# salesforce/ai-economist

Hardware: AMD Instinct MI355X
Metric: agent-steps/sec, gather-trade-build 25x25 4-agent batched envs (higher is better)
Workload: dtype u8/i32 state + f64 coin/utility (f32 observations); 1 GPU; C2 BASELINE configs[1]: gather-trade-build 25x25, 4 agents + planner, Build+CDA+Gather+PeriodicBracketTax, 4096 replicas/GPU, uniform random policy, planner not counted; envs_per_gpu=4096, global_envs=4096, n_agents=4, kernel_specialisation=compile time, parallelism=single GPU

## Files before the change

ai-economist_amd/csrc/aie_capi.hip:

```cpp
#include <hip/hip_runtime.h>

#include <cstdio>
#include <cstdlib>
#include <cstring>
#include <vector>

#include "aie_kernels.hip"
#include "aie_kernels_sampler.hip"
#include "aie_kernels_rollout.hip"
#include "aie_kernels_ose.hip"
#include "aie_kernels_saez.hip"
#include "aie_kernels_ppo.hip"
#include "aie_kernels_mlp.hip"
#include "aie_kernels_mlp_bwd.hip"
#include "aie_kernels_covid.hip"
#include "aie_jit.h"
#include "aie_trainer_plan.h"

struct aie_env {
  aie_params P{};
  aie_params* d_params;
  aie_tensor_table tt;
  uint8_t* arena;
  bool owns_arena;
// ... 206 lines not shown
  } else {
    k = AIE_KERNEL(aie_step_kernel);
  }
  if (!k.name) return AIE_E_INVALID;
  *out = {k, !k.fn, (unsigned)(covid ? AIE_NT : ose ? OSE_NT : 2 * AIE_NT), env->lds};
  return AIE_OK;
}

static int aie_launch_step(aie_env* env, const aie_route<aie_step_fn>& r, unsigned grid, const int32_t* d_actions_a,
                           const int32_t* d_actions_p, const NextActions& next, hipStream_t st) {
  if (r.module) {
    const aie_params* dp = env->d_params;
    uint8_t* ar = env->arena;
    NextActions nx = next;
    void* args[] = {&dp, &ar, &d_actions_a, &d_actions_p, &nx};
    AIE_HIP_CHECK(env, hipModuleLaunchKernel(env->jit_step, grid, 1, 1, r.block, 1, 1, (unsigned)r.lds, st, args, nullptr));
  } else {
    hipLaunchKernelGGL(r.k.fn, dim3(grid), dim3(r.block), r.lds, st, env->d_params, env->arena, d_actions_a, d_actions_p, next);
  }
  return AIE_OK;
}

static unsigned aie_log_grid(const aie_env* env) {
  if (env->P.c.scenario != AIE_SCN_GTB || env->P.ev_replicas <= 0 || !env->log_active) return 0;
  const int64_t L = env->P.ev_replicas, E8 = env->P.E >> 3;
  return (env->P.E & 7) ? (unsigned)L : (L <= E8 ? (unsigned)(8 * (L - 1) + 1) : (unsigned)env->P.E);
}

static aie_route<aie_reset_fn> aie_select_reset(const aie_env* env) {
  const aie_params& P = env->P;
  if (P.c.scenario == AIE_SCN_COVID) return {AIE_KERNEL(aie_covid_reset_kernel), false, AIE_NT, 0};
  if (P.c.scenario == AIE_SCN_ONE_STEP_ECONOMY) return {{nullptr, "aie_ose_reset_kernel"}, false, OSE_NT, env->lds};
  const bool layout = P.c.layout_gen != AIE_LAYOUT_FIXED;
  aie_route<aie_reset_fn> r = {AIE_KERNEL(aie_reset_kernel), false, AIE_NT, env->lds + aie::layout_gen_lds_bytes(P)};
  if (layout) r.k = AIE_KERNEL(aie_reset_kernel_layout), r.block = LG_NW * AIE_NT;
  if (P.dev_skip_mask == 0 && !env->dev_generic) {
    if (env->spec == AIE_KERNEL_INSTANCE_JIT) r.k = {nullptr, "aie_jit_reset"}, r.module = true;
    else if (env->spec >= 0 && env->spec < AIE_N_SPECS && aie_spec_kernel.reset[env->spec].fn) r.k = aie_spec_kernel.reset[env->spec];
  }
  return r;
}

static void aie_launch_reset(aie_env* env, const uint8_t* d_mask, int keep_rewards, void* stream) {
  const aie_route<aie_reset_fn> r = aie_select_reset(env);
  const dim3 g((unsigned)env->P.E), b(r.block);
  hipStream_t st = static_cast<hipStream_t>(stream);
  if (r.module) {
    const aie_params* dp = env->d_params;
    uint8_t* ar = env->arena;
    void* args[] = {&dp, &ar, &d_mask, &keep_rewards};
    (void)hipModuleLaunchKernel(env->jit_reset, g.x, 1, 1, b.x, 1, 1, (unsigned)r.lds, st, args, nullptr);
  } else if (!r.k.fn) {
    hipLaunchKernelGGL(aie_ose_reset_kernel, g, b, r.lds, st, env->d_params, env->arena, d_mask);
  } else {
    hipLaunchKernelGGL(r.k.fn, g, b, r.lds, st, env->d_params, env->arena, d_mask, keep_rewards);
  }
  if (env->P.c.scenario == AIE_SCN_GTB && aie__layout_staged(&env->P.c)) {
    const int threshold = env->P.E >= 4 ? (int)(env->P.E / 4) : 1;
    hipLaunchKernelGGL(aie_layout_decide_kernel, dim3(1), dim3(1), 0, st, env->d_params, env->arena, threshold);
    hipLaunchKernelGGL(aie_layout_refill_kernel, g, dim3(LG_NW * AIE_NT), r.lds, st, env->d_params, env->arena);
  }
}

template <bool LOGP>
using aie_policy_fn = void (*)(const aie_sampler_args, uint8_t*, const float*, const float*, uint64_t, int64_t, int32_t*, int32_t*,
                               int, const SamplerLogp<LOGP>);
template <bool LOGP>
static aie_policy_fn<LOGP> aie_policy_sampler(const aie_sampler_args& S) {
// ... 872 lines not shown
```

ai-economist_amd/csrc/aie_device.h:

```cpp
#pragma once
#include <hip/hip_runtime.h>
#include <stdint.h>

#include "aie_layout.h"
#include "aie_glibc_math.h"

#pragma clang fp contract(off)

#ifdef AIE_JIT
#include "aie_jit_image.h"
#else
#include "aie_spec_generated.h"
#endif
template <int SPEC>
__device__ __forceinline__ const aie_params& aie_spec_params(const aie_params* run_time) {
  if constexpr (SPEC < 0) return *run_time;
  else return *reinterpret_cast<const aie_params*>(aie_spec_image<SPEC>::bytes);
}

#define AIE_NT 64
#define AIE_DIRTY_CAP 64

namespace aie {

// ... 612 lines not shown
  return v;
}
__device__ __forceinline__ int rng_permutation(MTL& l, int lane, int n) {
  int p = lane;
  for (int i = n - 1; i >= 1; --i) {
    const int j = (int)rng_interval(l, lane, (uint32_t)i);
    const int vi = bcast(p, i), vj = bcast(p, j);
    p = (lane == i) ? vj : ((lane == j) ? vi : p);
  }
  return p;
}
__device__ __forceinline__ double rng_gauss(const Ctx& c, MT& m) {
  int32_t* has = R_I32(c, o_mt_has_gauss);
  double* g = R_F64(c, o_mt_gauss);
  if (*has) {
    const double t = *g;
    *has = 0;
    *g = 0.0;
    return t;
  }
  double f, x1, x2, r2;
  do {
    x1 = 2.0 * rng_double(m, c.tid) - 1.0;
    x2 = 2.0 * rng_double(m, c.tid) - 1.0;
    r2 = x1 * x1 + x2 * x2;
  } while (r2 >= 1.0 || r2 == 0.0);
  f = sqrt(-2.0 * aie_log_glibc(r2) / r2);
  *g = f * x1;
  *has = 1;
  return f * x2;
}
__device__ __forceinline__ double rng_pareto(MT& m, int lane, double a) { return aie_exp_glibc(-aie_log_glibc(1.0 - rng_double(m, lane)) / a) - 1.0; }
__device__ __forceinline__ double rng_lognormal(const Ctx& c, MT& m, double mean, double sigma) { return aie_exp_glibc(mean + sigma * rng_gauss(c, m)); }

#pragma clang fp contract(off)
__device__ __forceinline__ double tax_curr_rate_max(const Ctx& c) {
  return aie_annealed_tax_limit(*R_I32(c, o_tax_last_completions), c.R.c.tax_annealing_warmup,
                                c.R.c.tax_annealing_slope, c.R.c.tax_rate_max);
}
__device__ __forceinline__ uint8_t* saez_block(const Ctx& c) {
  return C_MET(c) - c.R.a_metrics - (int64_t)c.e * c.P.met_bytes + c.R.a_saez + (int64_t)c.e * c.P.saez_stride;
}
__device__ __forceinline__ double tax_rate(const Ctx& c, int b) {
  if (c.P.c.tax_model == AIE_TAX_MODEL_WRAPPER) return c.rtab[R_I32(c, o_tax_rate_idx)[b]];
  if (c.saez) {
    const double r = R_F64(c, o_tax_saez_rates)[b];
    const double cap = c.P.c.tax_annealing ? tax_curr_rate_max(c) : c.R.c.tax_rate_max;
    return r < cap ? r : cap;
  }
  const double r = c.R.c.tax_fixed_rates[b];
  if (!c.P.c.tax_annealing) return r;
  const double cap = tax_curr_rate_max(c);
  return r < cap ? r : cap;
}
__device__ __forceinline__ double tax_rate_obs(const Ctx& c, int b) {
  if (c.saez) return R_F64(c, o_tax_saez_obs_rates)[b];
  return tax_rate(c, b);
}
__device__ __forceinline__ bool tax_rate_action_visible(const Ctx& c, int j) {
  if (!c.P.c.tax_annealing) return true;
  double full = 0;
  for (int k = 0; k < c.P.c.tax_n_disc_rates; ++k) full = fmax(full, fabs(c.rtab[k]));
  const double vis = aie_annealed_tax_limit(*R_I32(c, o_tax_last_completions), c.R.c.tax_annealing_warmup,
                                            c.R.c.tax_annealing_slope, full);
  return fabs(c.rtab[j]) <= vis;
}
// ... 67 lines not shown
```

ai-economist_amd/csrc/aie_kernels.hip:

```cpp
#pragma once
#include "aie_device.h"

namespace aie {
__device__ __forceinline__ bool can_agent_occupy(const Ctx& c, int r, int col, int agent) {
  if (r < 0 || r >= c.P.H || col < 0 || col >= c.P.W) return false;
  const int cell = r * c.P.W + col;
  const uint32_t w = R_CELLS(c)[cell];
  if (AIE_CELL_FLAGS(w) & AIE_CELL_WATER) return false;
  const int o = AIE_CELL_OWNER(w);
  if (!(o < 0 || o == agent)) return false;
  const int occ = c.locmap[cell];
  return occ == 0 || occ == agent + 1;
}

__device__ __forceinline__ void log_event(const Ctx& c, int type, int a1, int a2, int a3, int a4, int a5,
                                          int a6, int a7, int a8, double f) {
  if (c.tid != 0) return;
  const int k = c.srcn[2];
  if (k >= c.R.ev_cap) return;
  int32_t* row = c.ev + 4 + k * AIE_EV_WORDS;
  row[0] = type; row[1] = a1; row[2] = a2; row[3] = a3; row[4] = a4;
  row[5] = a5; row[6] = a6; row[7] = a7; row[8] = a8; row[9] = 0;
  *reinterpret_cast<double*>(row + 10) = f;
  c.srcn[2] = k + 1;
// ... 1106 lines not shown
  const uint32_t amap_bytes = (uint32_t)(n * c.P.am_ch * plane * 4), aidx_bytes = (uint32_t)(n * 2 * plane * 2);
  SpatialOut o;
  o.amap = make_rsrc(arena + c.R.a_obs_a_map + (int64_t)c.e * amap_bytes, amap_bytes);
  o.aidx = make_rsrc(arena + c.R.a_obs_a_idx + (int64_t)c.e * aidx_bytes, aidx_bytes);
  const bool pl = c.P.c.planner_gets_spatial_info != 0;
  o.pmap = make_rsrc(arena + c.R.a_obs_p_map + (int64_t)c.e * CM * HW * 4, pl ? (uint32_t)(CM * HW * 4) : 0u);
  o.pidx = make_rsrc(arena + c.R.a_obs_p_idx + (int64_t)c.e * 2 * HW * 2, pl ? (uint32_t)(2 * HW * 2) : 0u);
  return o;
}

template <bool WATER>
__device__ __forceinline__ void crop_item(const Ctx& c, const SpatialOut& o, int i, int d, int r, int col) {
  constexpr int CM = WATER ? 6 : 5;
  const int H = c.P.H, W = c.P.W, WV2 = c.P.WV * c.P.WV;
  const int so = i * (CM + 1) * WV2 * 4, si = i * 2 * WV2 * 2;
  const bool in = (r >= 0) & (r < H) & (col >= 0) & (col < W);
  const int cell = in ? r * W + col : 0;
  const uint32_t cw = in ? R_CELLS(c)[cell] : 0x00ff0000u;
  float ch[6];
  cell_channels<WATER>(cw, ch);
#pragma unroll
  for (int k = 0; k < CM; ++k) buf_store_f32(o.amap, ch[k], 4 * d, so + k * WV2 * 4);
  buf_store_f32(o.amap, in ? 1.0f : 0.0f, 4 * d, so + CM * WV2 * 4);
  const int own = AIE_CELL_OWNER(cw);
  int v0 = own >= 0 ? own + 2 : 0;
  int v1 = in ? (int)c.locmap[cell] : 0;
  v1 = v1 ? v1 + 1 : 0;
  if (v0 == i + 2) v0 = 1;
  if (v1 == i + 2) v1 = 1;
  buf_store_i16(o.aidx, v0, 2 * d, si);
  buf_store_i16(o.aidx, v1, 2 * d, si + WV2 * 2);
}
template <bool WATER>
__device__ __forceinline__ void crop_agent(const Ctx& c, const SpatialOut& o, int i) {
  const int WV = c.P.WV, WV2 = WV * WV, w = c.P.c.obs_range;
  const int r0 = R_I32(c, o_loc_r)[i] - w, c0 = R_I32(c, o_loc_c)[i] - w;
  for (int d = c.tid; d < WV2; d += AIE_NT) {
    const int dr = udiv(d, WV, c.P.mg_WV), dc = d - dr * WV;
    crop_item<WATER>(c, o, i, d, r0 + dr, c0 + dc);
  }
}
template <bool WATER>
__device__ __forceinline__ void planner_cell(const Ctx& c, const SpatialOut& o, int cell) {
  constexpr int CM = WATER ? 6 : 5;
  const int HW = c.P.HW;
  float ch[6];
  const uint32_t cw = R_CELLS(c)[cell];
  cell_channels<WATER>(cw, ch);
#pragma unroll
  for (int k = 0; k < CM; ++k) buf_store_f32(o.pmap, ch[k], 4 * cell, k * HW * 4);
  const int own = AIE_CELL_OWNER(cw);
  const int occ = c.locmap[cell];
  buf_store_i16(o.pidx, own >= 0 ? own + 2 : 0, 2 * cell, 0);
  buf_store_i16(o.pidx, occ ? occ + 1 : 0, 2 * cell, HW * 2);
}

template <bool WATER>
__device__ __forceinline__ void write_spatial_observations_t(const Ctx& c, uint8_t* __restrict__ arena) {
  constexpr int CM = WATER ? 6 : 5;
  const int n = c.P.n, HW = c.P.HW;
  const uint32_t* cells = R_CELLS(c);
  const SpatialOut o = spatial_out<WATER>(c, arena);
  if (c.P.c.full_observability) {
    const uint32_t* lm4f = reinterpret_cast<const uint32_t*>(c.locmap);
    for (int i = 0; i < n; ++i) {
      const int so = i * CM * HW * 4, si = i * 2 * HW * 2;
      for (int q = c.tid; q < (HW >> 2); q += AIE_NT) {
        const uint4 cw = reinterpret_cast<const uint4*>(cells)[q];
        const uint32_t cws[4] = {cw.x, cw.y, cw.z, cw.w};
        float ch[4][6];
#pragma unroll
        for (int u = 0; u < 4; ++u) cell_channels<WATER>(cws[u], ch[u]);
#pragma unroll
        for (int k = 0; k < CM; ++k) buf_store_f32x4(o.amap, ch[0][k], ch[1][k], ch[2][k], ch[3][k], 16 * q, so + k * HW * 4);
        const uint32_t occ4 = lm4f[q];
#pragma unroll
        for (int u = 0; u < 4; ++u) {
          const int own = AIE_CELL_OWNER(cws[u]);
          int v0 = own >= 0 ? own + 2 : 0;
          const int occ = (int)((occ4 >> (8 * u)) & 0xffu);
          int v1 = occ ? occ + 1 : 0;
          if (v0 == i + 2) v0 = 1;
          if (v1 == i + 2) v1 = 1;
          buf_store_i16(o.aidx, v0, 8 * q + 2 * u, si);
          buf_store_i16(o.aidx, v1, 8 * q + 2 * u, si + HW * 2);
        }
      }
      for (int cell = 4 * (HW >> 2) + c.tid; cell < HW; cell += AIE_NT) {
        float ch[6];
        const uint32_t cw = cells[cell];
        cell_channels<WATER>(cw, ch);
#pragma unroll
        for (int k = 0; k < CM; ++k) buf_store_f32(o.amap, ch[k], 4 * cell, so + k * HW * 4);
        const int own = AIE_CELL_OWNER(cw);
        int v0 = own >= 0 ? own + 2 : 0;
        const int occ = c.locmap[cell];
        int v1 = occ ? occ + 1 : 0;
        if (v0 == i + 2) v0 = 1;
        if (v1 == i + 2) v1 = 1;
        buf_store_i16(o.aidx, v0, 2 * cell, si);
        buf_store_i16(o.aidx, v1, 2 * cell, si + HW * 2);
      }
    }
  } else {
    for (int i = 0; i < n; ++i) crop_agent<WATER>(c, o, i);
  }
  if (c.P.c.planner_gets_spatial_info) {
    const int nq4 = HW >> 2;
    const uint32_t* lm4 = reinterpret_cast<const uint32_t*>(c.locmap);
    for (int q = c.tid; q < nq4; q += AIE_NT) {
      const uint4 cw = reinterpret_cast<const uint4*>(cells)[q];
      const uint32_t cws[4] = {cw.x, cw.y, cw.z, cw.w};
      float ch[4][6];
#pragma unroll
      for (int u = 0; u < 4; ++u) cell_channels<WATER>(cws[u], ch[u]);
#pragma unroll
      for (int k = 0; k < CM; ++k) buf_store_f32x4(o.pmap, ch[0][k], ch[1][k], ch[2][k], ch[3][k], 16 * q, k * HW * 4);
      const uint32_t occ4 = lm4[q];
      uint32_t ow[2], oc[2];
#pragma unroll
      for (int u = 0; u < 4; ++u) {
        const int own = AIE_CELL_OWNER(cws[u]);
        const uint32_t vo = (uint32_t)(own >= 0 ? own + 2 : 0);
        const uint32_t occ = (occ4 >> (8 * u)) & 0xffu;
        const uint32_t vc = occ ? occ + 1 : 0;
        if (u & 1) { ow[u >> 1] |= vo << 16; oc[u >> 1] |= vc << 16; }
        else { ow[u >> 1] = vo; oc[u >> 1] = vc; }
      }
      buf_store_u32x2(o.pidx, ow[0], ow[1], 8 * q, 0);
      if ((HW & 1) == 0) {
        buf_store_u32x2(o.pidx, oc[0], oc[1], 8 * q, HW * 2);
      } else {
#pragma unroll
        for (int u = 0; u < 4; ++u) buf_store_i16(o.pidx, (int)((oc[u >> 1] >> (16 * (u & 1))) & 0xffffu), 8 * q + 2 * u, HW * 2);
      }
    }
    for (int cell = 4 * nq4 + c.tid; cell < HW; cell += AIE_NT) planner_cell<WATER>(c, o, cell);
  }
}

template <bool WATER>
__device__ __forceinline__ void agent_full_cell(const Ctx& c, const SpatialOut& o, int i, int cell) {
  constexpr int CM = WATER ? 6 : 5;
  const int HW = c.P.HW;
  const int so = i * CM * HW * 4, si = i * 2 * HW * 2;
  float ch[6];
  const uint32_t cw = R_CELLS(c)[cell];
  cell_channels<WATER>(cw, ch);
#pragma unroll
  for (int k = 0; k < CM; ++k) buf_store_f32(o.amap, ch[k], 4 * cell, so + k * HW * 4);
  const int own = AIE_CELL_OWNER(cw);
  int v0 = own >= 0 ? own + 2 : 0;
  const int occ = c.locmap[cell];
  int v1 = occ ? occ + 1 : 0;
  if (v0 == i + 2) v0 = 1;
  if (v1 == i + 2) v1 = 1;
  buf_store_i16(o.aidx, v0, 2 * cell, si);
  buf_store_i16(o.aidx, v1, 2 * cell, si + HW * 2);
}

template <bool WATER>
__device__ __forceinline__ void update_spatial_observations_t(const Ctx& c, uint8_t* __restrict__ arena) {
  const int n = c.P.n, W = c.P.W, WV = c.P.WV, w = c.P.c.obs_range;
  const int cnt = uni(c.dirty[0]);
  if (cnt > AIE_DIRTY_CAP) {
    write_spatial_observations_t<WATER>(c, arena);
    return;
  }
  const SpatialOut o = spatial_out<WATER>(c, arena);
  const uint32_t mv0 = (uint32_t)uni(c.dirty[1]), mv1 = (uint32_t)uni(c.dirty[2]);
  const uint16_t* dl = dirty_list(c);
  const int cell = c.tid < cnt ? (int)dl[c.tid] : -1;
  const int r = cell >= 0 ? udiv(cell, W, c.P.mg_W) : 0, col = cell - r * W;
  for (int i = 0; i < n; ++i) {
    if (c.P.c.full_observability) {
      if (cell >= 0) agent_full_cell<WATER>(c, o, i, cell);
      continue;
    }
    const bool moved = ((i < 32 ? mv0 >> i : mv1 >> (i - 32)) & 1u) != 0;
    if (moved) {
      crop_agent<WATER>(c, o, i);
    } else if (cell >= 0) {
      const int dr = r - (R_I32(c, o_loc_r)[i] - w), dc = col - (R_I32(c, o_loc_c)[i] - w);
      if (dr >= 0 && dr < WV && dc >= 0 && dc < WV) crop_item<WATER>(c, o, i, dr * WV + dc, r, col);
    }
  }
  if (c.P.c.planner_gets_spatial_info && cell >= 0) planner_cell<WATER>(c, o, cell);
}
__device__ __forceinline__ void write_spatial_observations(const Ctx& c, uint8_t* __restrict__ arena) {
  if (c.P.c.has_water) write_spatial_observations_t<true>(c, arena);
  else write_spatial_observations_t<false>(c, arena);
}
__device__ __forceinline__ void update_spatial_observations(const Ctx& c, uint8_t* __restrict__ arena) {
  if (c.P.c.has_water) update_spatial_observations_t<true>(c, arena);
  else update_spatial_observations_t<false>(c, arena);
}

__device__ __forceinline__ void flat_a(const BufRsrc& aflat, int idx, float v) { buf_store_f32(aflat, v, 4 * idx, 0); }

__device__ __forceinline__ float flat_time_value(const Ctx& c) {
  const int t = *R_I32(c, o_timestep);
  return (float)((double)t / (c.P.c.allow_observation_scaling ? (double)c.R.c.episode_length : 1.0));
}

struct AgentScalars {
  double coin; int inv0, inv1, lr, lc;
  __device__ __forceinline__ AgentScalars(const Ctx& c, int i)
      : coin(R_F64(c, o_inv_coin)[i]), inv0(R_I32(c, o_inv_res)[i]), inv1(R_I32(c, o_inv_res)[c.P.n + i]),
        lr(R_I32(c, o_loc_r)[i]), lc(R_I32(c, o_loc_c)[i]) {}
  __device__ __forceinline__ void write(const Ctx& c, uint8_t* __restrict__ arena, const BufRsrc& aflat, float* q, int i,
                                        float tval, double isc) const {
    const aie_params& P = c.P;
    const int f0 = i * P.FA;
    flat_a(aflat, f0 + P.fa_time, tval);
    const float w0 = (float)(coin * isc);
    const float w1 = (float)((double)inv0 * isc);
    const float w2 = (float)((double)inv1 * isc);
    const float w3 = (float)((double)lc / (double)P.W);
    const float w4 = (float)((double)lr / (double)P.H);
    flat_a(aflat, f0 + P.fa_world + 0, w0); flat_a(aflat, f0 + P.fa_world + 1, w1); flat_a(aflat, f0 + P.fa_world + 2, w2);
    if (!P.c.full_observability) {
      flat_a(aflat, f0 + P.fa_world + 3, w3); flat_a(aflat, f0 + P.fa_world + 4, w4);
      q[P.fpa_world + 0] = w0; q[P.fpa_world + 1] = w1; q[P.fpa_world + 2] = w2;
      if (P.c.planner_gets_spatial_info) { q[P.fpa_world + 3] = w3; q[P.fpa_world + 4] = w4; }
// ... 1054 lines not shown
        LG_ACC(4);
      }
    }
    happy = true;
    for (int q = 0; q < 2; ++q) {
      const int rs = q == 0 ? 1 : 0;
      int count = 0;
      for (int base = 0; base < HW; base += NT) {
        const int cell = base + gtid;
        count += lg_block_count(cell < HW && mbp[rs][cell], sh, par, wave, lane);
      }
      const double ratio = ((double)count / (double)HW) / c.R.c.layout_coverage[rs];
      if (!((1 / 1.4) <= ratio && ratio <= 1.4)) happy = false;
    }
  }
  mt_copy(m, s3.w[0]);
  m.pos = s3.pos;
  if (stage_out) {
    for (int cell = gtid; cell < HW; cell += NT) stage_out[cell] = (uint8_t)((mbp[0][cell] ? 1u : 0u) | (mbp[1][cell] ? 2u : 0u));
  } else {
    layout_install(c, gtid, NT, [&](int cell) -> uint32_t { return (mbp[0][cell] ? 1u : 0u) | (mbp[1][cell] ? 2u : 0u); });
  }
  __syncthreads();
#ifdef AIE_DEV
  if (c.R.dev_trace && gtid == 0) {
    lg_acc[0] = wall_clock64() - lg_start;
    for (int k = 0; k < 8; ++k) c.R.dev_trace[12 * c.e + k] = lg_acc[k];
  }
#endif
}
}

namespace aie {
template <int SPEC, bool LAYOUT = true>
__device__ __forceinline__ void reset_body(const aie_params* __restrict__ params, uint8_t* __restrict__ arena,
                                           const uint8_t* __restrict__ mask, int keep_rewards, uint8_t* lds) {
  const aie_params& R = *params;
  const aie_params& P = aie_spec_params<SPEC>(params);
  const int e = replica_of_block((int)blockIdx.x, R.E);
  if (mask && !mask[e]) return;
  const int gtid = (int)threadIdx.x, wave = gtid >> 6, nwaves = (int)blockDim.x >> 6;
  const Ctx c = make_ctx(P, R, lds, e, gtid & 63, arena);
  const int n = P.n, HW = P.HW, tid = c.tid;
  if (wave == 0) {
    for (int q = tid; q < (P.met_bytes >> 2); q += AIE_NT) reinterpret_cast<uint32_t*>(C_MET(c))[q] = 0u;
    if (c.ev && tid == 0) c.ev[0] = 0;
  }
  MT m;
  mt_init(m, P);
  load_record(c, arena, m, wave, nwaves, wave);
  __syncthreads();
  m.pos = uni(*R_I32(c, o_mt_pos));
  mt_fast_attach(c, m);
  if (LAYOUT && P.c.layout_gen != AIE_LAYOUT_FIXED) {
    if (aie__layout_staged(&P.c)) {
      uint32_t st[4];
#pragma unroll
      for (int k = 0; k < 4; ++k) st[k] = (uint32_t)uni((int)R_U32(c, o_mt)[k]);
      const uint64_t tag = aie_layout_tag(st);
      const uint64_t* tags = reinterpret_cast<const uint64_t*>(arena + R.a_layout_tag);
      int32_t* ctl = reinterpret_cast<int32_t*>(arena + R.a_layout_ctl);
      const uint64_t have = tags[e];
      const bool staged = (uint32_t)uni((int)(uint32_t)have) == (uint32_t)tag && (uint32_t)uni((int)(uint32_t)(have >> 32)) == (uint32_t)(tag >> 32);
      __syncthreads();
      if (staged) {
        const uint8_t* sp = arena + R.a_layout_stage + (int64_t)e * R.layout_stage_stride;
        layout_install(c, gtid, LG_NW * AIE_NT, [&](int cell) -> uint32_t { return sp[cell]; });
        __syncthreads();
      } else {
        LgShared* sh = lg_shared(lds + lds_bytes(P), P);
        if (gtid == 0) {
          sh->lhas = 0;
          sh->lcache = 0.0;
        }
        __syncthreads();
        uint32_t ks[2];
        aie_layout_stream(st, ks);
        MT ml;
        mt_init(ml, P);
        ml.fkey = ks[0];
        ml.fblk = 0xffffffffu;
        ml.fsalt = ks[1];
        layout_generate(c, ml, arena, lds + lds_bytes(P), gtid, &sh->lhas, &sh->lcache);
      }
      if (gtid == 0) {
        R_U32(c, o_mt)[3] = st[3] + 1u;
        atomicAdd(&ctl[0], 1);
        atomicAdd(&ctl[staged ? 2 : 3], 1);
      }
    } else {
      layout_generate(c, m, arena, lds + lds_bytes(P), gtid, R_I32(c, o_mt_has_gauss), R_F64(c, o_mt_gauss));
    }
    if (wave != 0) return;
  }
  {
    uint32_t* cells = R_CELLS(c);
    for (int q = tid; q < HW; q += AIE_NT) {
      const uint32_t fl = cells[q] >> 24;
      cells[q] = AIE_CELL_PACK((fl & AIE_CELL_STONE_SRC) ? 1 : 0, (fl & AIE_CELL_WOOD_SRC) ? 1 : 0, 0xff, fl);
    }
    if (tid < n) {
      R_I32(c, o_inv_res)[tid] = 0; R_I32(c, o_inv_res)[n + tid] = 0;
      R_I32(c, o_esc_res)[tid] = 0; R_I32(c, o_esc_res)[n + tid] = 0;
      R_F64(c, o_inv_coin)[tid] = c.R.c.starting_agent_coin;
      R_F64(c, o_esc_coin)[tid] = 0;
      R_F64(c, o_labor)[tid] = 0;
      R_I32(c, o_loc_r)[tid] = -1;
      R_I32(c, o_loc_c)[tid] = -1;
      if (!P.has_build) { R_F64(c, o_build_payment)[tid] = 0; R_F64(c, o_build_skill)[tid] = 0; }
      if (!P.has_gather) R_F64(c, o_bonus_gather_prob)[tid] = 0;
    }
    if (P.has_cda) {
      for (int q = tid; q < 2 * P.M; q += AIE_NT) { R_I32(c, o_cda_bids)[q] = 0; R_I32(c, o_cda_asks)[q] = 0; }
      for (int q = tid; q < 2 * n * P.P; q += AIE_NT) {
        R_U8(c, o_cda_bid_hist)[q] = 0; R_U8(c, o_cda_ask_hist)[q] = 0;
        R_F64(c, o_cda_price_history)[q] = 0;
      }
      for (int q = tid; q < 2 * n; q += AIE_NT) R_I32(c, o_cda_n_orders)[q] = 0;
      if (tid < 2) { R_I32(c, o_cda_n_bids)[tid] = 0; R_I32(c, o_cda_n_asks)[tid] = 0; }
    }
  }
  __syncthreads();
  build_src_list(c, arena);
  if (P.regen_conv) {
    const uint8_t* cb = reinterpret_cast<const uint8_t*>(R_CELLS(c));
    for (int q = tid; q < AIE_N_RES * HW; q += AIE_NT) {
      const int rs = q >= HW ? 1 : 0, cell = q - rs * HW, r0 = cell / P.W, c0 = cell - r0 * P.W;
      const int hw = P.c.regen_halfwidth[rs];
      const uint32_t bit = rs ? AIE_CELL_WOOD_SRC : AIE_CELL_STONE_SRC;
      int cnt = 0;
      for (int r = max(r0 - hw, 0); r <= min(r0 + hw, P.H - 1); ++r)
        for (int cc = max(c0 - hw, 0); cc <= min(c0 + hw, P.W - 1); ++cc)
          cnt += (cb[4 * (r * P.W + cc) + 3] & bit) ? 1 : 0;
      R_U8(c, o_regen_count)[q] = (uint8_t)cnt;
    }
  }
  rebuild_locmap(c);
  *R_I32(c, o_timestep) = 0;
  *R_I32(c, o_error_flags) = 0;
  const int place_perm = P.c.reset_random_order ? rng_permutation(m, tid, n) : tid;
  for (int k = 0; k < n; ++k) {
    const int i = bcast(place_perm, k);
    int r = (int)rng_interval(m, tid, (uint32_t)(P.H - 1)), col = (int)rng_interval(m, tid, (uint32_t)(P.W - 1)), tries = 0;
    while (!can_agent_occupy(c, r, col, i)) {
      r = (int)rng_interval(m, tid, (uint32_t)(P.H - 1));
      col = (int)rng_interval(m, tid, (uint32_t)(P.W - 1));
      if (++tries > 200) {
        *R_I32(c, o_error_flags) |= AIE_ERR_RESET_PLACEMENT;
        break;
      }
    }
    R_I32(c, o_loc_r)[i] = r;
    R_I32(c, o_loc_c)[i] = col;
    c.locmap[r * P.W + col] = (uint8_t)(i + 1);
  }
  for (int k = 0; k < P.c.n_components; ++k) {
    switch (P.c.components[k]) {
      case AIE_COMP_BUILD:
        for (int i = 0; i < n; ++i) {
          double skill = 1, pay = 1;
          const double pm = (double)c.R.c.build_payment_max_skill_multiplier;
          if (P.c.build_skill_dist == AIE_SKILL_PARETO) {
            skill = rng_pareto(m, tid, 4.0);
            pay = (pm - 1) * skill + 1; if (pm < pay) pay = pm;
          } else if (P.c.build_skill_dist == AIE_SKILL_LOGNORMAL) {
            skill = rng_lognormal(c, m, -1.0, 0.5);
            pay = (pm - 1) * skill + 1; if (pm < pay) pay = pm;
          }
          R_F64(c, o_build_payment)[i] = pay * (double)c.R.c.build_payment;
          R_F64(c, o_build_skill)[i] = skill;
        }
        break;
      case AIE_COMP_GATHER:
        for (int i = 0; i < n; ++i) {
          double b = 0.0;
          if (P.c.gather_skill_dist == AIE_SKILL_PARETO) { b = rng_pareto(m, tid, 3.0); b = (b < 2 ? b : 2) / 2; }
          else if (P.c.gather_skill_dist == AIE_SKILL_LOGNORMAL) { b = rng_lognormal(c, m, -2.022, 0.938); b = (b < 2 ? b : 2) / 2; }
          R_F64(c, o_bonus_gather_prob)[i] = b;
        }
        break;
      case AIE_COMP_TAX:
        for (int b = 0; b < P.NB; ++b) R_I32(c, o_tax_rate_idx)[b] = 0;
        *R_I32(c, o_tax_cycle_pos) = 1;
        for (int i = 0; i < n; ++i) {
          R_F64(c, o_tax_last_coin)[i] = R_F64(c, o_inv_coin)[i] + R_F64(c, o_esc_coin)[i];
          R_F64(c, o_tax_last_income)[i] = 0;
          R_F64(c, o_tax_last_marginal_rate)[i] = 0;
        }
        *R_F64(c, o_tax_total_collected) = 0;
        if (P.c.tax_model == AIE_TAX_SAEZ) {
          for (int b = 0; b < P.NB; ++b) R_F64(c, o_tax_saez_obs_rates)[b] = tax_rate(c, b);
          AIE_WSYNC();
          for (int b = 0; b < P.NB; ++b)
            R_F64(c, o_tax_saez_rates)[b] = reinterpret_cast<const double*>(saez_block(c) + AIE_SAEZ_OFF_AVG)[b];
        }
        break;
      default: break;
    }
  }
  if (P.c.fixed_four_skill_and_loc) {
    for (int i = 0; i < n; ++i) {
      c.locmap[R_I32(c, o_loc_r)[i] * P.W + R_I32(c, o_loc_c)[i]] = 0;
      R_I32(c, o_loc_r)[i] = -1;
      R_I32(c, o_loc_c)[i] = -1;
    }
    const int perm = rng_permutation(m, tid, n);
    for (int k = 0; k < n; ++k) {
      const int i = bcast(perm, k);
      const int r = c.R.c.ranked_locs[k][0], col = c.R.c.ranked_locs[k][1];
      if (can_agent_occupy(c, r, col, i)) {
        R_I32(c, o_loc_r)[i] = r;
        R_I32(c, o_loc_c)[i] = col;
        c.locmap[r * P.W + col] = (uint8_t)(i + 1);
      }
      R_F64(c, o_build_payment)[i] = c.R.c.avg_ranked_skill[k];
    }
  }
  if (P.c.split_water_line > 0) {
    for (int i = 0; i < n; ++i) {
      c.locmap[R_I32(c, o_loc_r)[i] * P.W + R_I32(c, o_loc_c)[i]] = 0;
      R_I32(c, o_loc_r)[i] = -1;
      R_I32(c, o_loc_c)[i] = -1;
    }
    const int perm = rng_permutation(m, tid, n);
    const int wl = P.c.split_water_line;
    for (int k = 0; k < n; ++k) {
      const int i = bcast(perm, k);
      R_F64(c, o_build_payment)[i] = c.R.c.avg_ranked_skill[k];
      const bool top = (c.R.c.split_top_ranks[k >> 5] >> (k & 31)) & 1u;
      const int r_min = top ? 0 : wl + 1, r_max = top ? wl : P.H;
      int r = r_min + (int)rng_interval(m, tid, (uint32_t)(r_max - r_min - 1));
      int col = (int)rng_interval(m, tid, (uint32_t)(P.W - 1)), tries = 0;
      while (!can_agent_occupy(c, r, col, i)) {
        r = r_min + (int)rng_interval(m, tid, (uint32_t)(r_max - r_min - 1));
        col = (int)rng_interval(m, tid, (uint32_t)(P.W - 1));
        if (++tries > 200) {
          *R_I32(c, o_error_flags) |= AIE_ERR_RESET_PLACEMENT;
          break;
        }
      }
      R_I32(c, o_loc_r)[i] = r;
      R_I32(c, o_loc_c)[i] = col;
      c.locmap[r * P.W + col] = (uint8_t)(i + 1);
    }
  }
  *R_I32(c, o_mt_pos) = m.pos;
  mt_fast_detach(c, m);
  __syncthreads();
  current_metrics(c);
  __syncthreads();
  if (tid <= n) R_F64(c, o_util)[tid] = scr_part(c)[tid];
  __syncthreads();
  write_spatial_observations(c, arena);
  if (tid == 0) *R_I32(c, o_obs_valid) = 1;
  write_flat_observations(c, arena);
  AIE_WSYNC();
  if (P.has_tax && P.c.tax_annealing && tid == 0) *R_I32(c, o_tax_last_completions) = *R_I32(c, o_completions);
  AIE_WSYNC();
  write_action_masks(c, arena);
  if (!keep_rewards) {
    if (tid < n) reinterpret_cast<float*>(arena + R.a_rew_a)[(int64_t)e * n + tid] = 0.0f;
    if (tid == 0) {
      reinterpret_cast<float*>(arena + R.a_rew_p)[e] = 0.0f;
      (arena + R.a_done)[e] = 0;
    }
  }
  __syncthreads();
  store_record(c, arena, m);
}
}

#ifndef AIE_JIT
extern "C" __global__ void __launch_bounds__(AIE_NT)
aie_reset_kernel(const aie_params* __restrict__ params, uint8_t* __restrict__ arena,
                 const uint8_t* __restrict__ mask, int keep_rewards) {
  extern __shared__ __attribute__((aligned(16))) uint8_t lds[];
  aie::reset_body<-1, false>(params, arena, mask, keep_rewards, lds);
}
extern "C" __global__ void __launch_bounds__(LG_NW * AIE_NT)
aie_reset_kernel_layout(const aie_params* __restrict__ params, uint8_t* __restrict__ arena,
                        const uint8_t* __restrict__ mask, int keep_rewards) {
  extern __shared__ __attribute__((aligned(16))) uint8_t lds[];
  aie::reset_body<-1, true>(params, arena, mask, keep_rewards, lds);
}
extern "C" __global__ void aie_layout_decide_kernel(const aie_params* __restrict__ params, uint8_t* __restrict__ arena, int threshold) {
  int32_t* ctl = reinterpret_cast<int32_t*>(arena + params->a_layout_ctl);
  const bool go = ctl[0] >= threshold;
  ctl[1] = go ? 1 : 0;
  if (go) ctl[0] = 0;
}
extern "C" __global__ void __launch_bounds__(LG_NW * AIE_NT)
aie_layout_refill_kernel(const aie_params* __restrict__ params, uint8_t* __restrict__ arena) {
  extern __shared__ __attribute__((aligned(16))) uint8_t lds[];
  const aie_params& P = *params;
  const int32_t* ctl = reinterpret_cast<const int32_t*>(arena + P.a_layout_ctl);
  if (!ctl[1]) return;
  const int e = (int)blockIdx.x, gtid = (int)threadIdx.x;
  const uint32_t* stg = reinterpret_cast<const uint32_t*>(arena + P.a_records + (int64_t)e * P.rec_bytes + P.o_mt);
  uint32_t st[4];
#pragma unroll
  for (int k = 0; k < 4; ++k) st[k] = (uint32_t)aie::uni((int)stg[k]);
  const uint64_t tag = aie_layout_tag(st);
  uint64_t* tags = reinterpret_cast<uint64_t*>(arena + P.a_layout_tag);
  const uint64_t have = tags[e];
  if ((uint32_t)aie::uni((int)(uint32_t)have) == (uint32_t)tag && (uint32_t)aie::uni((int)(uint32_t)(have >> 32)) == (uint32_t)(tag >> 32)) return;
  const aie::Ctx c = aie::make_ctx(P, P, lds, e, gtid & 63, arena);
// ... 86 lines not shown
```

Baseline: 778.9 million agent-steps/s.

## Run fixed-layout reset with multiple waves, offloading spatial observations to extra waves

The fixed-layout reset kernel now launches with LG_NW waves instead of one. The extra waves zero metrics and cells and write spatial observations in parallel, while wave 0 alone does placement, skills, metrics and record storage. Pareto skill sampling now draws all agents' values in one lane-parallel pass over the Mersenne Twister window instead of looping serially. Dev-only timing stamps are added. In exchange, larger blocks may lower occupancy, and the RNG consumption order must stay bit-identical.

```diff
diff --git a/ai-economist_amd/csrc/aie_capi.hip b/ai-economist_amd/csrc/aie_capi.hip
--- a/ai-economist_amd/csrc/aie_capi.hip
+++ b/ai-economist_amd/csrc/aie_capi.hip
@@ -262,8 +262,8 @@
   if (P.c.scenario == AIE_SCN_COVID) return {AIE_KERNEL(aie_covid_reset_kernel), false, AIE_NT, 0};
   if (P.c.scenario == AIE_SCN_ONE_STEP_ECONOMY) return {{nullptr, "aie_ose_reset_kernel"}, false, OSE_NT, env->lds};
   const bool layout = P.c.layout_gen != AIE_LAYOUT_FIXED;
-  aie_route<aie_reset_fn> r = {AIE_KERNEL(aie_reset_kernel), false, AIE_NT, env->lds + aie::layout_gen_lds_bytes(P)};
-  if (layout) r.k = AIE_KERNEL(aie_reset_kernel_layout), r.block = LG_NW * AIE_NT;
+  aie_route<aie_reset_fn> r = {AIE_KERNEL(aie_reset_kernel), false, LG_NW * AIE_NT, env->lds + aie::layout_gen_lds_bytes(P)};
+  if (layout) r.k = AIE_KERNEL(aie_reset_kernel_layout);
   if (P.dev_skip_mask == 0 && !env->dev_generic) {
     if (env->spec == AIE_KERNEL_INSTANCE_JIT) r.k = {nullptr, "aie_jit_reset"}, r.module = true;
     else if (env->spec >= 0 && env->spec < AIE_N_SPECS && aie_spec_kernel.reset[env->spec].fn) r.k = aie_spec_kernel.reset[env->spec];
diff --git a/ai-economist_amd/csrc/aie_device.h b/ai-economist_amd/csrc/aie_device.h
--- a/ai-economist_amd/csrc/aie_device.h
+++ b/ai-economist_amd/csrc/aie_device.h
@@ -668,6 +668,37 @@
 }
 __device__ __forceinline__ double rng_pareto(MT& m, int lane, double a) { return aie_exp_glibc(-aie_log_glibc(1.0 - rng_double(m, lane)) / a) - 1.0; }
 __device__ __forceinline__ double rng_lognormal(const Ctx& c, MT& m, double mean, double sigma) { return aie_exp_glibc(mean + sigma * rng_gauss(c, m)); }
+__device__ __forceinline__ uint32_t mt_window_word(const MT& m, int idx, int row_lo, int row_hi) {
+  uint32_t v = 0;
+#pragma unroll
+  for (int j = 0; j < 10; ++j) {
+    if (j < row_lo || j > row_hi) continue;
+    const uint32_t t = lane_get(m.r[j], idx & 63);
+    v = ((idx >> 6) == j) ? t : v;
+  }
+  return v;
+}
+__device__ __forceinline__ double rng_pareto_lanes(MT& m, int lane, int n, double a) {
+  if (m.pos >= AIE_MT_N) {
+    mt_twist(m, lane);
+    m.pos = 0;
+  }
+  const int p0 = m.pos, end = p0 + 2 * n, ia = p0 + 2 * lane;
+  const int last = (end < AIE_MT_N ? end : AIE_MT_N) - 1;
+  uint32_t wa = mt_window_word(m, ia, p0 >> 6, last >> 6), wb = mt_window_word(m, ia + 1, p0 >> 6, last >> 6);
+  if (end > AIE_MT_N) {
+    mt_twist(m, lane);
+    const int hi = (end - AIE_MT_N - 1) >> 6;
+    const uint32_t xa = mt_window_word(m, ia - AIE_MT_N, 0, hi), xb = mt_window_word(m, ia + 1 - AIE_MT_N, 0, hi);
+    wa = ia >= AIE_MT_N ? xa : wa;
+    wb = ia + 1 >= AIE_MT_N ? xb : wb;
+    m.pos = end - AIE_MT_N;
+  } else {
+    m.pos = end;
+  }
+  const double u = lane < n ? u53(mt_word(m, wa), mt_word(m, wb)) : 0.0;
+  return aie_exp_glibc(-aie_log_glibc(1.0 - u) / a) - 1.0;
+}
 
 #pragma clang fp contract(off)
 __device__ __forceinline__ double tax_curr_rate_max(const Ctx& c) {
diff --git a/ai-economist_amd/csrc/aie_kernels.hip b/ai-economist_amd/csrc/aie_kernels.hip
--- a/ai-economist_amd/csrc/aie_kernels.hip
+++ b/ai-economist_amd/csrc/aie_kernels.hip
@@ -1162,14 +1162,16 @@
   buf_store_i16(o.aidx, v1, 2 * d, si + WV2 * 2);
 }
 template <bool WATER>
-__device__ __forceinline__ void crop_agent(const Ctx& c, const SpatialOut& o, int i) {
+__device__ __forceinline__ void crop_agent(const Ctx& c, const SpatialOut& o, int i, int t0, int nt) {
   const int WV = c.P.WV, WV2 = WV * WV, w = c.P.c.obs_range;
   const int r0 = R_I32(c, o_loc_r)[i] - w, c0 = R_I32(c, o_loc_c)[i] - w;
-  for (int d = c.tid; d < WV2; d += AIE_NT) {
+  for (int d = t0; d < WV2; d += nt) {
     const int dr = udiv(d, WV, c.P.mg_WV), dc = d - dr * WV;
     crop_item<WATER>(c, o, i, d, r0 + dr, c0 + dc);
   }
 }
+template <bool WATER>
+__device__ __forceinline__ void crop_agent(const Ctx& c, const SpatialOut& o, int i) { crop_agent<WATER>(c, o, i, c.tid, AIE_NT); }
 template <bool WATER>
 __device__ __forceinline__ void planner_cell(const Ctx& c, const SpatialOut& o, int cell) {
   constexpr int CM = WATER ? 6 : 5;
@@ -1186,7 +1188,7 @@
 }
 
 template <bool WATER>
-__device__ __forceinline__ void write_spatial_observations_t(const Ctx& c, uint8_t* __restrict__ arena) {
+__device__ __forceinline__ void write_spatial_observations_t(const Ctx& c, uint8_t* __restrict__ arena, int t0, int nt) {
   constexpr int CM = WATER ? 6 : 5;
   const int n = c.P.n, HW = c.P.HW;
   const uint32_t* cells = R_CELLS(c);
@@ -1195,7 +1197,7 @@
     const uint32_t* lm4f = reinterpret_cast<const uint32_t*>(c.locmap);
     for (int i = 0; i < n; ++i) {
       const int so = i * CM * HW * 4, si = i * 2 * HW * 2;
-      for (int q = c.tid; q < (HW >> 2); q += AIE_NT) {
+      for (int q = t0; q < (HW >> 2); q += nt) {
         const uint4 cw = reinterpret_cast<const uint4*>(cells)[q];
         const uint32_t cws[4] = {cw.x, cw.y, cw.z, cw.w};
         float ch[4][6];
@@ -1216,7 +1218,7 @@
           buf_store_i16(o.aidx, v1, 8 * q + 2 * u, si + HW * 2);
         }
       }
-      for (int cell = 4 * (HW >> 2) + c.tid; cell < HW; cell += AIE_NT) {
+      for (int cell = 4 * (HW >> 2) + t0; cell < HW; cell += nt) {
         float ch[6];
         const uint32_t cw = cells[cell];
         cell_channels<WATER>(cw, ch);
@@ -1233,12 +1235,12 @@
       }
     }
   } else {
-    for (int i = 0; i < n; ++i) crop_agent<WATER>(c, o, i);
+    for (int i = 0; i < n; ++i) crop_agent<WATER>(c, o, i, t0, nt);
   }
   if (c.P.c.planner_gets_spatial_info) {
     const int nq4 = HW >> 2;
     const uint32_t* lm4 = reinterpret_cast<const uint32_t*>(c.locmap);
-    for (int q = c.tid; q < nq4; q += AIE_NT) {
+    for (int q = t0; q < nq4; q += nt) {
       const uint4 cw = reinterpret_cast<const uint4*>(cells)[q];
       const uint32_t cws[4] = {cw.x, cw.y, cw.z, cw.w};
       float ch[4][6];
@@ -1265,8 +1267,13 @@
         for (int u = 0; u < 4; ++u) buf_store_i16(o.pidx, (int)((oc[u >> 1] >> (16 * (u & 1))) & 0xffffu), 8 * q + 2 * u, HW * 2);
       }
     }
-    for (int cell = 4 * nq4 + c.tid; cell < HW; cell += AIE_NT) planner_cell<WATER>(c, o, cell);
-  }
+    for (int cell = 4 * nq4 + t0; cell < HW; cell += nt) planner_cell<WATER>(c, o, cell);
+  }
+}
+
+template <bool WATER>
+__device__ __forceinline__ void write_spatial_observations_t(const Ctx& c, uint8_t* __restrict__ arena) {
+  write_spatial_observations_t<WATER>(c, arena, c.tid, AIE_NT);
 }
 
 template <bool WATER>
@@ -1320,6 +1327,10 @@
 __device__ __forceinline__ void write_spatial_observations(const Ctx& c, uint8_t* __restrict__ arena) {
   if (c.P.c.has_water) write_spatial_observations_t<true>(c, arena);
   else write_spatial_observations_t<false>(c, arena);
+}
+__device__ __forceinline__ void write_spatial_observations(const Ctx& c, uint8_t* __restrict__ arena, int t0, int nt) {
+  if (c.P.c.has_water) write_spatial_observations_t<true>(c, arena, t0, nt);
+  else write_spatial_observations_t<false>(c, arena, t0, nt);
 }
 __device__ __forceinline__ void update_spatial_observations(const Ctx& c, uint8_t* __restrict__ arena) {
   if (c.P.c.has_water) update_spatial_observations_t<true>(c, arena);
@@ -2440,6 +2451,19 @@
 }
 
 namespace aie {
+#ifdef AIE_DEV
+#define RS_STAMP(k)                                               \
+  do {                                                            \
+    if (rs_on) {                                                  \
+      asm volatile("s_waitcnt vmcnt(0) lgkmcnt(0)" ::: "memory"); \
+      const uint64_t rs_now = wall_clock64();                     \
+      if (gtid == 0) c.R.dev_trace[12 * c.e + (k)] = rs_now - rs_t; \
+      rs_t = rs_now;                                              \
+    }                                                             \
+  } while (0)
+#else
+#define RS_STAMP(k) do { } while (0)
+#endif
 template <int SPEC, bool LAYOUT = true>
 __device__ __forceinline__ void reset_body(const aie_params* __restrict__ params, uint8_t* __restrict__ arena,
                                            const uint8_t* __restrict__ mask, int keep_rewards, uint8_t* lds) {
@@ -2450,16 +2474,23 @@
   const int gtid = (int)threadIdx.x, wave = gtid >> 6, nwaves = (int)blockDim.x >> 6;
   const Ctx c = make_ctx(P, R, lds, e, gtid & 63, arena);
   const int n = P.n, HW = P.HW, tid = c.tid;
-  if (wave == 0) {
-    for (int q = tid; q < (P.met_bytes >> 2); q += AIE_NT) reinterpret_cast<uint32_t*>(C_MET(c))[q] = 0u;
-    if (c.ev && tid == 0) c.ev[0] = 0;
-  }
+  const bool fixed = !(LAYOUT && P.c.layout_gen != AIE_LAYOUT_FIXED);
+  const int nw = fixed ? nwaves : 1;
+  const int lt = fixed ? gtid : tid, lnt = nw * AIE_NT;
+#ifdef AIE_DEV
+  const bool rs_on = c.R.dev_trace && P.c.layout_gen == AIE_LAYOUT_FIXED;
+  const uint64_t rs_start = wall_clock64();
+  uint64_t rs_t = rs_start;
+#endif
+  for (int q = gtid; q < (P.met_bytes >> 2); q += nwaves * AIE_NT) reinterpret_cast<uint32_t*>(C_MET(c))[q] = 0u;
+  if (c.ev && gtid == 0) c.ev[0] = 0;
   MT m;
   mt_init(m, P);
-  load_record(c, arena, m, wave, nwaves, wave);
+  load_record(c, arena, m, wave, nwaves, fixed ? 0 : wave);
   __syncthreads();
   m.pos = uni(*R_I32(c, o_mt_pos));
-  mt_fast_attach(c, m);
+  if (!fixed || wave == 0) mt_fast_attach(c, m);
+  RS_STAMP(0);
   if (LAYOUT && P.c.layout_gen != AIE_LAYOUT_FIXED) {
     if (aie__layout_staged(&P.c)) {
       uint32_t st[4];
@@ -2503,11 +2534,11 @@
   }
   {
     uint32_t* cells = R_CELLS(c);
-    for (int q = tid; q < HW; q += AIE_NT) {
+    for (int q = lt; q < HW; q += lnt) {
       const uint32_t fl = cells[q] >> 24;
       cells[q] = AIE_CELL_PACK((fl & AIE_CELL_STONE_SRC) ? 1 : 0, (fl & AIE_CELL_WOOD_SRC) ? 1 : 0, 0xff, fl);
     }
-    if (tid < n) {
+    if (lt < n) {
       R_I32(c, o_inv_res)[tid] = 0; R_I32(c, o_inv_res)[n + tid] = 0;
       R_I32(c, o_esc_res)[tid] = 0; R_I32(c, o_esc_res)[n + tid] = 0;
       R_F64(c, o_inv_coin)[tid] = c.R.c.starting_agent_coin;
@@ -2519,20 +2550,21 @@
       if (!P.has_gather) R_F64(c, o_bonus_gather_prob)[tid] = 0;
     }
     if (P.has_cda) {
-      for (int q = tid; q < 2 * P.M; q += AIE_NT) { R_I32(c, o_cda_bids)[q] = 0; R_I32(c, o_cda_asks)[q] = 0; }
-      for (int q = tid; q < 2 * n * P.P; q += AIE_NT) {
+      for (int q = lt; q < 2 * P.M; q += lnt) { R_I32(c, o_cda_bids)[q] = 0; R_I32(c, o_cda_asks)[q] = 0; }
+      for (int q = lt; q < 2 * n * P.P; q += lnt) {
         R_U8(c, o_cda_bid_hist)[q] = 0; R_U8(c, o_cda_ask_hist)[q] = 0;
         R_F64(c, o_cda_price_history)[q] = 0;
       }
-      for (int q = tid; q < 2 * n; q += AIE_NT) R_I32(c, o_cda_n_orders)[q] = 0;
-      if (tid < 2) { R_I32(c, o_cda_n_bids)[tid] = 0; R_I32(c, o_cda_n_asks)[tid] = 0; }
+      for (int q = lt; q < 2 * n; q += lnt) R_I32(c, o_cda_n_orders)[q] = 0;
+      if (lt < 2) { R_I32(c, o_cda_n_bids)[tid] = 0; R_I32(c, o_cda_n_asks)[tid] = 0; }
     }
   }
   __syncthreads();
-  build_src_list(c, arena);
+  RS_STAMP(1);
+  if (wave == 0 && (P.c.layout_gen != AIE_LAYOUT_FIXED || !P.c.shared_layout)) build_src_list(c, arena);
   if (P.regen_conv) {
     const uint8_t* cb = reinterpret_cast<const uint8_t*>(R_CELLS(c));
-    for (int q = tid; q < AIE_N_RES * HW; q += AIE_NT) {
+    for (int q = lt; q < AIE_N_RES * HW; q += lnt) {
       const int rs = q >= HW ? 1 : 0, cell = q - rs * HW, r0 = cell / P.W, c0 = cell - r0 * P.W;
       const int hw = P.c.regen_halfwidth[rs];
       const uint32_t bit = rs ? AIE_CELL_WOOD_SRC : AIE_CELL_STONE_SRC;
@@ -2543,104 +2575,17 @@
       R_U8(c, o_regen_count)[q] = (uint8_t)cnt;
     }
   }
-  rebuild_locmap(c);
-  *R_I32(c, o_timestep) = 0;
-  *R_I32(c, o_error_flags) = 0;
-  const int place_perm = P.c.reset_random_order ? rng_permutation(m, tid, n) : tid;
-  for (int k = 0; k < n; ++k) {
-    const int i = bcast(place_perm, k);
-    int r = (int)rng_interval(m, tid, (uint32_t)(P.H - 1)), col = (int)rng_interval(m, tid, (uint32_t)(P.W - 1)), tries = 0;
-    while (!can_agent_occupy(c, r, col, i)) {
-      r = (int)rng_interval(m, tid, (uint32_t)(P.H - 1));
-      col = (int)rng_interval(m, tid, (uint32_t)(P.W - 1));
-      if (++tries > 200) {
-        *R_I32(c, o_error_flags) |= AIE_ERR_RESET_PLACEMENT;
-        break;
-      }
-    }
-    R_I32(c, o_loc_r)[i] = r;
-    R_I32(c, o_loc_c)[i] = col;
-    c.locmap[r * P.W + col] = (uint8_t)(i + 1);
-  }
-  for (int k = 0; k < P.c.n_components; ++k) {
-    switch (P.c.components[k]) {
-      case AIE_COMP_BUILD:
-        for (int i = 0; i < n; ++i) {
-          double skill = 1, pay = 1;
-          const double pm = (double)c.R.c.build_payment_max_skill_multiplier;
-          if (P.c.build_skill_dist == AIE_SKILL_PARETO) {
-            skill = rng_pareto(m, tid, 4.0);
-            pay = (pm - 1) * skill + 1; if (pm < pay) pay = pm;
-          } else if (P.c.build_skill_dist == AIE_SKILL_LOGNORMAL) {
-            skill = rng_lognormal(c, m, -1.0, 0.5);
-            pay = (pm - 1) * skill + 1; if (pm < pay) pay = pm;
-          }
-          R_F64(c, o_build_payment)[i] = pay * (double)c.R.c.build_payment;
-          R_F64(c, o_build_skill)[i] = skill;
-        }
-        break;
-      case AIE_COMP_GATHER:
-        for (int i = 0; i < n; ++i) {
-          double b = 0.0;
-          if (P.c.gather_skill_dist == AIE_SKILL_PARETO) { b = rng_pareto(m, tid, 3.0); b = (b < 2 ? b : 2) / 2; }
-          else if (P.c.gather_skill_dist == AIE_SKILL_LOGNORMAL) { b = rng_lognormal(c, m, -2.022, 0.938); b = (b < 2 ? b : 2) / 2; }
-          R_F64(c, o_bonus_gather_prob)[i] = b;
-        }
-        break;
-      case AIE_COMP_TAX:
-        for (int b = 0; b < P.NB; ++b) R_I32(c, o_tax_rate_idx)[b] = 0;
-        *R_I32(c, o_tax_cycle_pos) = 1;
-        for (int i = 0; i < n; ++i) {
-          R_F64(c, o_tax_last_coin)[i] = R_F64(c, o_inv_coin)[i] + R_F64(c, o_esc_coin)[i];
-          R_F64(c, o_tax_last_income)[i] = 0;
-          R_F64(c, o_tax_last_marginal_rate)[i] = 0;
-        }
-        *R_F64(c, o_tax_total_collected) = 0;
-        if (P.c.tax_model == AIE_TAX_SAEZ) {
-          for (int b = 0; b < P.NB; ++b) R_F64(c, o_tax_saez_obs_rates)[b] = tax_rate(c, b);
-          AIE_WSYNC();
-          for (int b = 0; b < P.NB; ++b)
-            R_F64(c, o_tax_saez_rates)[b] = reinterpret_cast<const double*>(saez_block(c) + AIE_SAEZ_OFF_AVG)[b];
-        }
-        break;
-      default: break;
-    }
-  }
-  if (P.c.fixed_four_skill_and_loc) {
-    for (int i = 0; i < n; ++i) {
-      c.locmap[R_I32(c, o_loc_r)[i] * P.W + R_I32(c, o_loc_c)[i]] = 0;
-      R_I32(c, o_loc_r)[i] = -1;
-      R_I32(c, o_loc_c)[i] = -1;
-    }
-    const int perm = rng_permutation(m, tid, n);
+  if (wave == 0) {
+    rebuild_locmap(c);
+    RS_STAMP(2);
+    *R_I32(c, o_timestep) = 0;
+    *R_I32(c, o_error_flags) = 0;
+    const int place_perm = P.c.reset_random_order ? rng_permutation(m, tid, n) : tid;
     for (int k = 0; k < n; ++k) {
-      const int i = bcast(perm, k);
-      const int r = c.R.c.ranked_locs[k][0], col = c.R.c.ranked_locs[k][1];
-      if (can_agent_occupy(c, r, col, i)) {
-        R_I32(c, o_loc_r)[i] = r;
-        R_I32(c, o_loc_c)[i] = col;
-        c.locmap[r * P.W + col] = (uint8_t)(i + 1);
-      }
-      R_F64(c, o_build_payment)[i] = c.R.c.avg_ranked_skill[k];
-    }
-  }
-  if (P.c.split_water_line > 0) {
-    for (int i = 0; i < n; ++i) {
-      c.locmap[R_I32(c, o_loc_r)[i] * P.W + R_I32(c, o_loc_c)[i]] = 0;
-      R_I32(c, o_loc_r)[i] = -1;
-      R_I32(c, o_loc_c)[i] = -1;
-    }
-    const int perm = rng_permutation(m, tid, n);
-    const int wl = P.c.split_water_line;
-    for (int k = 0; k < n; ++k) {
-      const int i = bcast(perm, k);
-      R_F64(c, o_build_payment)[i] = c.R.c.avg_ranked_skill[k];
-      const bool top = (c.R.c.split_top_ranks[k >> 5] >> (k & 31)) & 1u;
-      const int r_min = top ? 0 : wl + 1, r_max = top ? wl : P.H;
-      int r = r_min + (int)rng_interval(m, tid, (uint32_t)(r_max - r_min - 1));
-      int col = (int)rng_interval(m, tid, (uint32_t)(P.W - 1)), tries = 0;
+      const int i = bcast(place_perm, k);
+      int r = (int)rng_interval(m, tid, (uint32_t)(P.H - 1)), col = (int)rng_interval(m, tid, (uint32_t)(P.W - 1)), tries = 0;
       while (!can_agent_occupy(c, r, col, i)) {
-        r = r_min + (int)rng_interval(m, tid, (uint32_t)(r_max - r_min - 1));
+        r = (int)rng_interval(m, tid, (uint32_t)(P.H - 1));
         col = (int)rng_interval(m, tid, (uint32_t)(P.W - 1));
         if (++tries > 200) {
           *R_I32(c, o_error_flags) |= AIE_ERR_RESET_PLACEMENT;
@@ -2651,18 +2596,137 @@
       R_I32(c, o_loc_c)[i] = col;
       c.locmap[r * P.W + col] = (uint8_t)(i + 1);
     }
-  }
-  *R_I32(c, o_mt_pos) = m.pos;
-  mt_fast_detach(c, m);
+    RS_STAMP(3);
+    for (int k = 0; k < P.c.n_components; ++k) {
+      switch (P.c.components[k]) {
+        case AIE_COMP_BUILD:
+          if (P.c.build_skill_dist == AIE_SKILL_PARETO) {
+            const double pm = (double)c.R.c.build_payment_max_skill_multiplier;
+            const double skill = rng_pareto_lanes(m, tid, n, 4.0);
+            double pay = (pm - 1) * skill + 1; if (pm < pay) pay = pm;
+            if (tid < n) {
+              R_F64(c, o_build_payment)[tid] = pay * (double)c.R.c.build_payment;
+              R_F64(c, o_build_skill)[tid] = skill;
+            }
+            AIE_WSYNC();
+            break;
+          }
+          for (int i = 0; i < n; ++i) {
+            double skill = 1, pay = 1;
+            const double pm = (double)c.R.c.build_payment_max_skill_multiplier;
+            if (P.c.build_skill_dist == AIE_SKILL_LOGNORMAL) {
+              skill = rng_lognormal(c, m, -1.0, 0.5);
+              pay = (pm - 1) * skill + 1; if (pm < pay) pay = pm;
+            }
+            R_F64(c, o_build_payment)[i] = pay * (double)c.R.c.build_payment;
+            R_F64(c, o_build_skill)[i] = skill;
+          }
+          break;
+        case AIE_COMP_GATHER:
+          if (P.c.gather_skill_dist == AIE_SKILL_PARETO) {
+            double b = rng_pareto_lanes(m, tid, n, 3.0);
+            b = (b < 2 ? b : 2) / 2;
+            if (tid < n) R_F64(c, o_bonus_gather_prob)[tid] = b;
+            AIE_WSYNC();
+            break;
+          }
+          for (int i = 0; i < n; ++i) {
+            double b = 0.0;
+            if (P.c.gather_skill_dist == AIE_SKILL_LOGNORMAL) { b = rng_lognormal(c, m, -2.022, 0.938); b = (b < 2 ? b : 2) / 2; }
+            R_F64(c, o_bonus_gather_prob)[i] = b;
+          }
+          break;
+        case AIE_COMP_TAX:
+          for (int b = 0; b < P.NB; ++b) R_I32(c, o_tax_rate_idx)[b] = 0;
+          *R_I32(c, o_tax_cycle_pos) = 1;
+          for (int i = 0; i < n; ++i) {
+            R_F64(c, o_tax_last_coin)[i] = R_F64(c, o_inv_coin)[i] + R_F64(c, o_esc_coin)[i];
+            R_F64(c, o_tax_last_income)[i] = 0;
+            R_F64(c, o_tax_last_marginal_rate)[i] = 0;
+          }
+          *R_F64(c, o_tax_total_collected) = 0;
+          if (P.c.tax_model == AIE_TAX_SAEZ) {
+            for (int b = 0; b < P.NB; ++b) R_F64(c, o_tax_saez_obs_rates)[b] = tax_rate(c, b);
+            AIE_WSYNC();
+            for (int b = 0; b < P.NB; ++b)
+              R_F64(c, o_tax_saez_rates)[b] = reinterpret_cast<const double*>(saez_block(c) + AIE_SAEZ_OFF_AVG)[b];
+          }
+          break;
+        default: break;
+      }
+    }
+    if (P.c.fixed_four_skill_and_loc) {
+      for (int i = 0; i < n; ++i) {
+        c.locmap[R_I32(c, o_loc_r)[i] * P.W + R_I32(c, o_loc_c)[i]] = 0;
+        R_I32(c, o_loc_r)[i] = -1;
+        R_I32(c, o_loc_c)[i] = -1;
+      }
+      const int perm = rng_permutation(m, tid, n);
+      for (int k = 0; k < n; ++k) {
+        const int i = bcast(perm, k);
+        const int r = c.R.c.ranked_locs[k][0], col = c.R.c.ranked_locs[k][1];
+        if (can_agent_occupy(c, r, col, i)) {
+          R_I32(c, o_loc_r)[i] = r;
+          R_I32(c, o_loc_c)[i] = col;
+          c.locmap[r * P.W + col] = (uint8_t)(i + 1);
+        }
+        R_F64(c, o_build_payment)[i] = c.R.c.avg_ranked_skill[k];
+      }
+    }
+    if (P.c.split_water_line > 0) {
+      for (int i = 0; i < n; ++i) {
+        c.locmap[R_I32(c, o_loc_r)[i] * P.W + R_I32(c, o_loc_c)[i]] = 0;
+        R_I32(c, o_loc_r)[i] = -1;
+        R_I32(c, o_loc_c)[i] = -1;
+      }
+      const int perm = rng_permutation(m, tid, n);
+      const int wl = P.c.split_water_line;
+      for (int k = 0; k < n; ++k) {
+        const int i = bcast(perm, k);
+        R_F64(c, o_build_payment)[i] = c.R.c.avg_ranked_skill[k];
+        const bool top = (c.R.c.split_top_ranks[k >> 5] >> (k & 31)) & 1u;
+        const int r_min = top ? 0 : wl + 1, r_max = top ? wl : P.H;
+        int r = r_min + (int)rng_interval(m, tid, (uint32_t)(r_max - r_min - 1));
+        int col = (int)rng_interval(m, tid, (uint32_t)(P.W - 1)), tries = 0;
+        while (!can_agent_occupy(c, r, col, i)) {
+          r = r_min + (int)rng_interval(m, tid, (uint32_t)(r_max - r_min - 1));
+          col = (int)rng_interval(m, tid, (uint32_t)(P.W - 1));
+          if (++tries > 200) {
+            *R_I32(c, o_error_flags) |= AIE_ERR_RESET_PLACEMENT;
+            break;
+          }
+        }
+        R_I32(c, o_loc_r)[i] = r;
+        R_I32(c, o_loc_c)[i] = col;
+        c.locmap[r * P.W + col] = (uint8_t)(i + 1);
+      }
+    }
+    *R_I32(c, o_mt_pos) = m.pos;
+    mt_fast_detach(c, m);
+  }
   __syncthreads();
+  if (wave != 0) {
+    write_spatial_observations(c, arena, lt - AIE_NT, lnt - AIE_NT);
+#ifdef AIE_DEV
+    if (rs_on) {
+      asm volatile("s_waitcnt vmcnt(0) lgkmcnt(0)" ::: "memory");
+      if (gtid == AIE_NT) c.R.dev_trace[12 * c.e + 11] = wall_clock64() - rs_t;
+    }
+#endif
+    return;
+  }
+  RS_STAMP(4);
   current_metrics(c);
-  __syncthreads();
+  AIE_WSYNC();
   if (tid <= n) R_F64(c, o_util)[tid] = scr_part(c)[tid];
-  __syncthreads();
-  write_spatial_observations(c, arena);
+  AIE_WSYNC();
+  RS_STAMP(5);
+  if (nw == 1) write_spatial_observations(c, arena);
   if (tid == 0) *R_I32(c, o_obs_valid) = 1;
+  RS_STAMP(6);
   write_flat_observations(c, arena);
   AIE_WSYNC();
+  RS_STAMP(7);
   if (P.has_tax && P.c.tax_annealing && tid == 0) *R_I32(c, o_tax_last_completions) = *R_I32(c, o_completions);
   AIE_WSYNC();
   write_action_masks(c, arena);
@@ -2673,13 +2737,18 @@
       (arena + R.a_done)[e] = 0;
     }
   }
-  __syncthreads();
+  AIE_WSYNC();
+  RS_STAMP(8);
   store_record(c, arena, m);
+  RS_STAMP(9);
+#ifdef AIE_DEV
+  if (rs_on && gtid == 0) c.R.dev_trace[12 * c.e + 10] = wall_clock64() - rs_start;
+#endif
 }
 }
 
 #ifndef AIE_JIT
-extern "C" __global__ void __launch_bounds__(AIE_NT)
+extern "C" __global__ void __launch_bounds__(LG_NW * AIE_NT)
 aie_reset_kernel(const aie_params* __restrict__ params, uint8_t* __restrict__ arena,
                  const uint8_t* __restrict__ mask, int keep_rewards) {
   extern __shared__ __attribute__((aligned(16))) uint8_t lds[];
```

After: 785.7 million agent-steps/s (median of 6 runs). Within noise of the previous version (+0.9%).
